# HoangChuongNguyen/ibgs

Hardware: AMD Instinct MI355X
Metric: train-step fps (fwd+bwd raster) @1080p, 1M Gaussians (higher is better)
Workload: dtype f32

## Files before the change

ibgs_amd/csrc/api.hip:

```cpp
#include "common.h"
#include "sh_color.h"
#include <sched.h>
#include <time.h>
#include <string.h>
#include <cstdlib>
#include <stdlib.h>
#include <stdio.h>
#include <cstdarg>
#include <cstdio>
#include <cstring>
#include <vector>
#include <map>
#include <mutex>

namespace ibgs {

static thread_local char g_err[512] = "";
void set_error(const char* fmt, ...)
{
    va_list ap; va_start(ap, fmt);
    vsnprintf(g_err, sizeof(g_err), fmt, ap);
    va_end(ap);
}

// ... 464 lines not shown
    if (a.render_geo) {
        if (a.plane_mode == IBGS_PLANE_NONE ? (!a.all_map || !a.dL_dall_map)
                                            : (a.plane_mode == IBGS_PLANE_LEARNT ? (!a.plane_normal || !a.dL_dplane_normal)
                                                                                 : (a.plane_mode != IBGS_PLANE_SMALLEST_AXIS || !a.scales || !a.rotations))) {
            set_error("geo backward: plane inputs / gradient outputs missing"); return -IBGS_ERR_INVALID;
        }
        if (!a.out_depth || !a.out_warped || !a.ref_to_src || !a.src_images) { set_error("geo backward inputs missing"); return -IBGS_ERR_INVALID; }
        if (!a.tex || a.tex_bytes < ibgs_required_tex(a.n_src, a.W, a.H)) { set_error("tex scratch too small"); return -IBGS_ERR_ALLOC; }
        if (!a.geo_table || a.geo_table_bytes < (a.buffer_length > 0 ? ibgs_required_geo_table_for(a.W, a.H, a.buffer_length) : ibgs_required_geo_table(a.W, a.H))) { set_error("geo_table scratch too small"); return -IBGS_ERR_ALLOC; }
    }
    int rc;
    GeomState g = GeomState::carve(a.geom, (size_t)a.P, nullptr);
    ImgState im = ImgState::carve(a.img, a.W, a.H, nullptr);
    BinState b = BinState::carve(a.binning, (size_t)a.R, a.W, a.H, nullptr);
    const float4* rgba = nullptr;
    float* geo_tab = nullptr;
    if (a.render_geo) {
        float4* t = reinterpret_cast<float4*>((reinterpret_cast<uintptr_t>(a.tex) + 127) & ~uintptr_t(127));
        const bool window = a.dL_ddepth || a.dL_dwarped;
        if (window && !(a.flags & IBGS_FLAG_TEX_PACKED) && (rc = launch_pack_rgba(s, a.src_images, t, a.W, a.H, a.n_src))) return rc;
        rgba = t;
        geo_tab = reinterpret_cast<float*>((reinterpret_cast<uintptr_t>(a.geo_table) + 127) & ~uintptr_t(127));
    }
    if (a.R > 0) {
        const bool det = (a.flags & IBGS_FLAG_DETERMINISTIC) != 0;
        DetState ds{};
        int ipt = 1;
        if (det) {
            if (!a.det_scratch || a.det_scratch_bytes < ibgs_required_deterministic_for(a.R, a.P, a.W, a.H, a.render_geo, a.flags)) { set_error("det_scratch too small"); return -IBGS_ERR_ALLOC; }
            ipt = render_backward_waves_per_tile(a);
            ds = DetState::carve(a.det_scratch, (size_t)a.R * ipt, (size_t)a.P, nullptr);
            if ((rc = launch_det_prepare(s, ds, (size_t)a.R * ipt))) return rc;
        }
        if ((rc = launch_render_backward(s, a, g, b, im, rgba, det ? ds.slab : nullptr, geo_tab))) return rc;
        if (det) { StageTimer t(s, IBGS_STAGE_TILE_ORDER); if ((rc = launch_det_reduce(s, ds, b.point_list, (size_t)a.R, ipt, a.P, a.grad_acc, g.offsets + a.P))) return rc; }
        if ((rc = stage_check(s, debug, "render backward"))) return rc;
    }
    { StageTimer t(s, IBGS_STAGE_PREPROCESS_BWD); if ((rc = launch_preprocess_backward(s, a, g))) return rc; }
    if ((rc = stage_check(s, debug, "preprocess backward"))) return rc;
    return check_sort_flag(rs, true);
}

int32_t ibgs_sh_grad_from_views(void* stream, int32_t P, int32_t D, int32_t M, int32_t n_views, const float* means3D,
                                const float* camposes, const float* dcolor, int64_t view_stride, float* dL_dsh)
{
    if (view_stride == 0) view_stride = (int64_t)P * 3;
    if (view_stride < (int64_t)P * 3) { set_error("view_stride smaller than P x 3"); return -IBGS_ERR_INVALID; }
    if (P <= 0 || M <= 0) return 0;
    if (D < 0 || D > 3 || (D + 1) * (D + 1) > M || n_views < 0) { set_error("bad SH degree / view count"); return -IBGS_ERR_INVALID; }
    if (!means3D || !dL_dsh || (n_views > 0 && (!camposes || !dcolor))) { set_error("null pointer"); return -IBGS_ERR_INVALID; }
    return launch_sh_grad_from_views(reinterpret_cast<hipStream_t>(stream), P, D, M, n_views, means3D, camposes, dcolor, (size_t)view_stride, dL_dsh);
}

int32_t ibgs_mark_visible(void* stream, int32_t P, const float* means3D, const float* viewmatrix,
                          const float* projmatrix, uint8_t* present)
{
    (void)projmatrix;
    if (P <= 0) return 0;
    if (!means3D || !viewmatrix || !present) { set_error("null pointer"); return -IBGS_ERR_INVALID; }
    return launch_mark_visible(reinterpret_cast<hipStream_t>(stream), P, means3D, viewmatrix, present);
}
// ... 3 lines not shown
```

ibgs_amd/csrc/common.h:

```cpp
#pragma once
#include <hip/hip_runtime.h>
#include <stdint.h>
#include <stddef.h>
#include <stdlib.h>
#include "../../include/ibgs_rast.h"

namespace ibgs {

constexpr int TILE = IBGS_TILE;
constexpr int WAVE = 64;
constexpr int REC_FLOATS = 16;
constexpr int GACC_FLOATS = 16;
constexpr bool grad_acc_offsets_fit32(long long P) { return P >= 0 && P <= (1ll << 32) / (long long)(GACC_FLOATS * sizeof(float)); }

constexpr int IBGS_CULL_WORDS = 4;
constexpr int IBGS_CULL_MAX_TILES = 64 * IBGS_CULL_WORDS;

enum RecField { R_X = 0, R_Y = 1, R_OP = 2, R_PAD0 = 3, R_CA = 4, R_CB = 5, R_CC = 6, R_DIST = 7,
                R_R = 8, R_G = 9, R_B = 10, R_PAD1 = 11, R_NX = 12, R_NY = 13, R_NZ = 14, R_PAD2 = 15 };

enum GaccField { G_SX = 0, G_SY = 1, G_AX = 2, G_AY = 3, G_SXX = 4, G_SXY = 5, G_SYY = 6, G_S0 = 7,
                 G_R = 8, G_G = 9, G_B = 10, G_NX = 11, G_NY = 12, G_NZ = 13, G_DIST = 14, G_PAD = 15 };

struct Carver {
// ... 330 lines not shown
                     uint32_t* result_alt = nullptr, const ShRide* ride = nullptr);
bool radix_takes_sh_ride(size_t n, int nbits);
void radix_set_sh_ride(bool on);
size_t radix_zero_elems(size_t n, int nbits);
int exclusive_scan_u32(hipStream_t s, const uint32_t* in, uint32_t* out, size_t n, uint32_t* scratch,
                       size_t scratch_elems, bool with_total);
size_t scan_scratch_elems(size_t n);
int radix_set_onesweep(int mode);
void radix_set_lookback_spins(uint32_t v);

int launch_binning(hipStream_t s, int P, int64_t cap, int gx, int gy, const GeomState& g, const BinState& b, uint32_t* ranges,
                   const uint32_t* order_hint = nullptr, uint32_t* meta = nullptr ,
                   int n_views = 1 ,
                   const uint32_t* sort_flag = nullptr, uint32_t* host_note = nullptr ,
                   uint32_t note_ticket = 0 );
constexpr int ORDER_CLASSES = 1024;
int launch_binning_scatter(hipStream_t s, int64_t cap, int gx, int gy, const BinState& b);

int launch_pack_rgba(hipStream_t s, const float* src, float4* dst, int W, int H, int n);
constexpr int GEO_TAB_FIELDS = 6;
inline size_t geo_table_floats(int W, int H) { return (size_t)W * H * IBGS_MAX_BUFFER_LENGTH * GEO_TAB_FIELDS; }
int launch_render_forward(hipStream_t s, const ibgs_forward_args& a, const GeomState& g, const BinState& b,
                          const ImgState& im, const float4* src_rgba);
int launch_render_backward(hipStream_t s, const ibgs_backward_args& a, const GeomState& g, const BinState& b,
                           const ImgState& im, const float4* src_rgba, float* slab = nullptr, float* geo_tab = nullptr);
int launch_preprocess_backward(hipStream_t s, const ibgs_backward_args& a, const GeomState& g);

struct DetState {
    float* slab;
    uint32_t* keys[2];
    uint32_t* vals[2];
    uint32_t* seg;
    uint32_t* hist; size_t hist_elems;
    static DetState carve(char* base, size_t rows, size_t P, size_t* total);
};
int render_backward_waves_per_tile(const ibgs_backward_args& a);
int render_backward_ref_arith(uint32_t flags);
int launch_det_prepare(hipStream_t s, const DetState& d, size_t rows);
int launch_det_reduce(hipStream_t s, const DetState& d, const uint32_t* point_list, size_t R, int ipt, int P, float* gacc, const uint32_t* listed );
int launch_sh_grad_from_views(hipStream_t s, int P, int D, int M, int n_views, const float* means3D, const float* camposes,
                              const float* dcolor, size_t view_stride, float* dL_dsh);

__device__ __forceinline__ uint32_t pack_rect(int lo, int hi) { return (uint32_t)lo | ((uint32_t)hi << 16); }

}
```

ibgs_amd/csrc/preprocess_bwd.hip:

```cpp
#include "common.h"
#include "adam_math.h"

namespace ibgs {

__constant__ float bC1 = 0.4886025119029199f;
__constant__ float bC0 = 0.28209479177387814f;
__constant__ float bC2[5] = {1.0925484305920792f, -1.0925484305920792f, 0.31539156525252005f,
                             -1.0925484305920792f, 0.5462742152960396f};
__constant__ float bC3[7] = {-0.5900435899266435f, 2.890611442640554f, -0.4570457994644658f,
                             0.3731763325901154f, -0.4570457994644658f, 1.445305721320277f,
                             -0.5900435899266435f};

struct PreBwdParams {
    int P, D, M;
    const float* means3D; const int32_t* radii; const float* shs; const float* shs_rest; const uint8_t* clamped;
    const float* scales; const float* rotations; float scale_modifier;
    const float* cov3D;
    float* gacc;
    int clear_gacc;
    int risky_rows;
    const float* rec;
    float* dL_dmean2D; float* dL_dmean2D_abs; float* dL_dconic; float* dL_dopacity; float* dL_dcolors;
    float* dL_dall_map; float* dL_dmean3D; float* dL_dcov3D; float* dL_dsh; float* dL_dsh_rest; float* dL_dscale; float* dL_drot;
    const float* plane_normal; const float* plane_offset; int plane_mode;
    float* dL_dplane_normal; float* dL_dplane_offset;
};

__device__ __forceinline__ int sh_basis(int D, float x, float y, float z, float (&B)[16])
{
    int nb = 1;
    B[0] = bC0;
    const float xx = x * x, yy = y * y, zz = z * z, xy = x * y, yz = y * z, xz = x * z;
    if (D > 0) {
        B[1] = -bC1 * y; B[2] = bC1 * z; B[3] = -bC1 * x; nb = 4;
        if (D > 1) {
            B[4] = bC2[0] * xy; B[5] = bC2[1] * yz; B[6] = bC2[2] * (2.0f * zz - xx - yy);
            B[7] = bC2[3] * xz; B[8] = bC2[4] * (xx - yy); nb = 9;
            if (D > 2) {
                B[9] = bC3[0] * y * (3.0f * xx - yy); B[10] = bC3[1] * xy * z;
                B[11] = bC3[2] * y * (4.0f * zz - xx - yy);
                B[12] = bC3[3] * z * (2.0f * zz - 3.0f * xx - 3.0f * yy);
                B[13] = bC3[4] * x * (4.0f * zz - xx - yy); B[14] = bC3[5] * z * (xx - yy);
                B[15] = bC3[6] * x * (xx - 3.0f * yy); nb = 16;
            }
        }
    }
    return nb;
}

template <bool FAST16, bool WRITE_SH, bool SPLIT = false>
__global__ void __launch_bounds__(FAST16 ? 64 : 256) preprocess_bwd_kernel(PreBwdParams p, Cam cam)
{
    __shared__ float4 s_t[FAST16 ? 64 * 13 : 1];
    const int i = blockIdx.x * blockDim.x + threadIdx.x;
    const bool valid = i < p.P;
    bool vis = valid && (p.radii[i] > 0);
    float4 g0 = make_float4(0.f, 0.f, 0.f, 0.f), g1 = g0, g2 = g0, g3 = g0;
    if (vis) {
        float4* grow = reinterpret_cast<float4*>(p.gacc + (size_t)i * GACC_FLOATS);
        g0 = grow[0]; g1 = grow[1]; g2 = grow[2]; g3 = grow[3];
        const uint32_t any = (__float_as_uint(g0.x) | __float_as_uint(g0.y) | __float_as_uint(g0.z) | __float_as_uint(g0.w) |
                              __float_as_uint(g1.x) | __float_as_uint(g1.y) | __float_as_uint(g1.z) | __float_as_uint(g1.w) |
                              __float_as_uint(g2.x) | __float_as_uint(g2.y) | __float_as_uint(g2.z) | __float_as_uint(g2.w) |
                              __float_as_uint(g3.x) | __float_as_uint(g3.y) | __float_as_uint(g3.z) | __float_as_uint(g3.w)) & 0x7FFFFFFFu;
        if (any == 0u) vis = false;
        else if (p.clear_gacc) { const float4 z = make_float4(0.f, 0.f, 0.f, 0.f); grow[0] = z; grow[1] = z; grow[2] = z; grow[3] = z; }
    }
    float gv[(FAST16 && WRITE_SH) ? 48 : 1];
    if (FAST16 && WRITE_SH) {
#pragma unroll
        for (int k = 0; k < 48; k++) gv[k] = 0.f;
    }
    if (valid && !vis) {
        p.dL_dmean2D[3 * i] = 0.f; p.dL_dmean2D[3 * i + 1] = 0.f; p.dL_dmean2D[3 * i + 2] = 0.f;
        if (p.dL_dmean2D_abs) { p.dL_dmean2D_abs[3 * i] = 0.f; p.dL_dmean2D_abs[3 * i + 1] = 0.f; p.dL_dmean2D_abs[3 * i + 2] = 0.f; }
        if (p.dL_dconic) { p.dL_dconic[4 * i] = 0.f; p.dL_dconic[4 * i + 1] = 0.f; p.dL_dconic[4 * i + 2] = 0.f; p.dL_dconic[4 * i + 3] = 0.f; }
        p.dL_dopacity[i] = 0.f;
        if (p.dL_dcolors) { p.dL_dcolors[3 * i] = 0.f; p.dL_dcolors[3 * i + 1] = 0.f; p.dL_dcolors[3 * i + 2] = 0.f; }
        if (p.dL_dall_map) for (int k = 0; k < 5; k++) p.dL_dall_map[5 * i + k] = 0.f;
        if (p.dL_dplane_normal) { p.dL_dplane_normal[3 * i] = 0.f; p.dL_dplane_normal[3 * i + 1] = 0.f; p.dL_dplane_normal[3 * i + 2] = 0.f; }
        if (p.dL_dplane_offset) p.dL_dplane_offset[i] = 0.f;
        p.dL_dmean3D[3 * i] = 0.f; p.dL_dmean3D[3 * i + 1] = 0.f; p.dL_dmean3D[3 * i + 2] = 0.f;
        if (p.dL_dcov3D) for (int k = 0; k < 6; k++) p.dL_dcov3D[6 * i + k] = 0.f;
        if (!FAST16 && WRITE_SH && p.shs) {
            if (SPLIT) {
                float* gd = p.dL_dsh + (size_t)i * 3; float* gr = p.dL_dsh_rest + (size_t)i * (p.M - 1) * 3;
                gd[0] = gd[1] = gd[2] = 0.f;
                for (int k = 0; k < 3 * (p.M - 1); k++) gr[k] = 0.f;
            } else { float* gsh = p.dL_dsh + (size_t)i * p.M * 3; for (int k = 0; k < 3 * p.M; k++) gsh[k] = 0.f; }
        }
        if (p.scales) {
            p.dL_dscale[3 * i] = 0.f; p.dL_dscale[3 * i + 1] = 0.f; p.dL_dscale[3 * i + 2] = 0.f;
            p.dL_drot[4 * i] = 0.f; p.dL_drot[4 * i + 1] = 0.f; p.dL_drot[4 * i + 2] = 0.f; p.dL_drot[4 * i + 3] = 0.f;
        }
    }
    if (FAST16 && SPLIT && p.shs) {
// ... 280 lines not shown
#pragma unroll
        for (int r = 0; r < 3; r++) p.dL_dscale[3 * i + r] = R[0][r] * dM[r][0] + R[1][r] * dM[r][1] + R[2][r] * dM[r][2];
#pragma unroll
        for (int r = 0; r < 3; r++)
#pragma unroll
            for (int cc = 0; cc < 3; cc++) G[r][cc] = sv[r] * dM[r][cc];
        p.dL_drot[4 * i + 0] = prot[0] + 2 * z * (G[0][1] - G[1][0]) + 2 * y * (G[2][0] - G[0][2]) + 2 * x * (G[1][2] - G[2][1]);
        p.dL_drot[4 * i + 1] = prot[1] + 2 * y * (G[1][0] + G[0][1]) + 2 * z * (G[2][0] + G[0][2]) + 2 * r_ * (G[1][2] - G[2][1]) - 4 * x * (G[2][2] + G[1][1]);
        p.dL_drot[4 * i + 2] = prot[2] + 2 * x * (G[1][0] + G[0][1]) + 2 * r_ * (G[2][0] - G[0][2]) + 2 * z * (G[1][2] + G[2][1]) - 4 * y * (G[2][2] + G[0][0]);
        p.dL_drot[4 * i + 3] = prot[3] + 2 * r_ * (G[0][1] - G[1][0]) + 2 * x * (G[2][0] + G[0][2]) + 2 * y * (G[1][2] + G[2][1]) - 4 * z * (G[1][1] + G[0][0]);
    }
    }

    if (FAST16 && WRITE_SH && SPLIT && p.shs) {
        const int lane = threadIdx.x;
        __syncthreads();
        float* s_w = reinterpret_cast<float*>(s_t);
        s_w[2880 + 3 * lane] = gv[0]; s_w[2880 + 3 * lane + 1] = gv[1]; s_w[2880 + 3 * lane + 2] = gv[2];
#pragma unroll
        for (int k = 0; k < 45; k++) s_w[45 * lane + k] = gv[3 + k];
        __syncthreads();
        const int i0 = blockIdx.x * 64;
        const int nrows = min(64, p.P - i0);
        float4* dr = reinterpret_cast<float4*>(p.dL_dsh_rest + (size_t)i0 * 45);
        float4* dd = reinterpret_cast<float4*>(p.dL_dsh + (size_t)i0 * 3);
#pragma unroll
        for (int it = 0; it < 12; it++) {
            const int q = it * 64 + lane;
            const float4 f4 = s_t[q];
            const float f[4] = {f4.x, f4.y, f4.z, f4.w};
            if (q < 720) {
                if (4 * q + 3 < nrows * 45) dr[q] = f4;
                else { float* op = p.dL_dsh_rest + (size_t)i0 * 45; for (int k = 0; k < 4; k++) if (4 * q + k < nrows * 45) op[4 * q + k] = f[k]; }
            } else {
                const int qd = q - 720;
                if (4 * qd + 3 < nrows * 3) dd[qd] = f4;
                else { float* op = p.dL_dsh + (size_t)i0 * 3; for (int k = 0; k < 4; k++) if (4 * qd + k < nrows * 3) op[4 * qd + k] = f[k]; }
            }
        }
    } else if (FAST16 && WRITE_SH && p.shs) {
        const int lane = threadIdx.x;
#pragma unroll
        for (int v = 0; v < 12; v++) s_t[lane * 13 + v] = make_float4(gv[4 * v], gv[4 * v + 1], gv[4 * v + 2], gv[4 * v + 3]);
        __syncthreads();
        const int i0 = blockIdx.x * 64;
        const int nrows = min(64, p.P - i0);
        float4* dst = reinterpret_cast<float4*>(p.dL_dsh + (size_t)i0 * 48);
#pragma unroll
        for (int k = 0; k < 12; k++) {
            const int f = lane + 64 * k;
            const int r = f / 12, c = f - 12 * r;
            if (r < nrows) dst[f] = s_t[r * 13 + c];
        }
    }
}

int launch_preprocess_backward(hipStream_t s, const ibgs_backward_args& a, const GeomState& g)
{
    PreBwdParams p;
    p.P = a.P; p.D = a.D; p.M = a.M;
    p.means3D = a.means3D; p.radii = a.radii; p.shs = a.shs; p.shs_rest = a.shs_rest; p.clamped = g.clamped;
    p.scales = a.scales; p.rotations = a.rotations; p.scale_modifier = a.scale_modifier;
    p.cov3D = a.cov3D_precomp ? a.cov3D_precomp : g.cov3D;
    p.gacc = a.grad_acc; p.rec = g.rec; p.clear_gacc = (a.flags & IBGS_FLAG_CLEAR_GRAD_ACC) ? 1 : 0;
    { const int ra = render_backward_ref_arith(a.flags); p.risky_rows = (ra & 4) ? 2 : ((ra & 2) ? 1 : 0); }
    p.dL_dmean2D = a.dL_dmean2D; p.dL_dmean2D_abs = a.dL_dmean2D_abs; p.dL_dconic = a.dL_dconic;
    p.dL_dopacity = a.dL_dopacity; p.dL_dcolors = a.dL_dcolors; p.dL_dall_map = a.dL_dall_map;
    p.dL_dmean3D = a.dL_dmean3D; p.dL_dcov3D = a.dL_dcov3D; p.dL_dsh = a.dL_dsh; p.dL_dsh_rest = a.dL_dsh_rest; p.dL_dscale = a.dL_dscale; p.dL_drot = a.dL_drot;
    p.plane_normal = a.plane_normal; p.plane_offset = a.plane_offset; p.plane_mode = a.plane_mode;
    p.dL_dplane_normal = a.dL_dplane_normal; p.dL_dplane_offset = a.dL_dplane_offset;
    const Cam cam = make_cam(a.viewmatrix, a.projmatrix, a.campos, a.bg, a.tanfovx, a.tanfovy, a.W, a.H);
    const bool factored = a.shs && (a.flags & IBGS_FLAG_SH_FACTORED);
    const bool split = a.shs && a.shs_rest;
    if (a.shs && a.M == 16) {
        if (factored && split) hipLaunchKernelGGL((preprocess_bwd_kernel<true, false, true>), dim3((a.P + 63) / 64), dim3(64), 0, s, p, cam);
        else if (factored) hipLaunchKernelGGL((preprocess_bwd_kernel<true, false>), dim3((a.P + 63) / 64), dim3(64), 0, s, p, cam);
        else if (split) hipLaunchKernelGGL((preprocess_bwd_kernel<true, true, true>), dim3((a.P + 63) / 64), dim3(64), 0, s, p, cam);
        else hipLaunchKernelGGL((preprocess_bwd_kernel<true, true>), dim3((a.P + 63) / 64), dim3(64), 0, s, p, cam);
    } else {
        if (factored && split) hipLaunchKernelGGL((preprocess_bwd_kernel<false, false, true>), dim3((a.P + 255) / 256), dim3(256), 0, s, p, cam);
        else if (factored) hipLaunchKernelGGL((preprocess_bwd_kernel<false, false>), dim3((a.P + 255) / 256), dim3(256), 0, s, p, cam);
        else if (split) hipLaunchKernelGGL((preprocess_bwd_kernel<false, true, true>), dim3((a.P + 255) / 256), dim3(256), 0, s, p, cam);
        else hipLaunchKernelGGL((preprocess_bwd_kernel<false, true>), dim3((a.P + 255) / 256), dim3(256), 0, s, p, cam);
    }
    IBGS_HIP(hipGetLastError());
    return 0;
}

template <bool FAST16>
__global__ void __launch_bounds__(FAST16 ? 64 : 256) sh_grad_from_views_kernel(int P, int D, int M, int n_views, size_t view_stride, const float* __restrict__ means3D,
                                                                                const float* __restrict__ camposes, const float* __restrict__ dcolor,
                                                                                float* __restrict__ dL_dsh)
{
// ... 144 lines not shown
```

ibgs_amd/csrc/render_bwd.hip:

```cpp
#include "common.h"
#include <stdlib.h>
#include "wave_reduce.h"
#include <type_traits>

namespace ibgs {

struct BwdParams {
    const uint32_t* ranges; const uint32_t* point_list; const float4* rec;
    Cam cam;
    int ntiles;
    TileMap tmap;
    int n_src; int tex_quant;
    int power_skip;
    const uint32_t* tile_risky;
    const float* ref_to_src; const float4* src_rgba;
    const float* final_T; const uint32_t* n_contrib; const float* sum_w; const uint32_t* low_high;
    const int32_t* valid_idx; const float* valid_w;
    const float* depth_pixels; const float* warped_pixels;
    const float* dL_dcolor; const float* dL_dnormal; const float* dL_ddepth; const float* dL_dwarped;
    float* gacc;
    int tab_slots;
    const uint32_t* slot_c; const uint32_t* meta; float* tab;
    const uint32_t* order;
    int slab_ipt;
    int hybrid_grid1;
    int acc32;
    float* slab;
};

__device__ __forceinline__ float quant8b(float a, int quant) { return quant ? floorf(a * 256.0f + 0.5f) * (1.0f / 256.0f) : a; }

__device__ __forceinline__ float4 tex_rgba_b(const float4* __restrict__ img, int W, int H, float x, float y, int quant)
{
#pragma clang fp contract(off)
    const float xb = x - 0.5f, yb = y - 0.5f;
    const float fxi = floorf(xb), fyi = floorf(yb);
    const float a = quant8b(xb - fxi, quant), b = quant8b(yb - fyi, quant);
    const int i0 = min(W - 1, max(0, (int)fxi)), i1 = min(W - 1, max(0, (int)fxi + 1));
    const int j0 = min(H - 1, max(0, (int)fyi)), j1 = min(H - 1, max(0, (int)fyi + 1));
    const float4 t00 = img[(size_t)j0 * W + i0], t10 = img[(size_t)j0 * W + i1];
    const float4 t01 = img[(size_t)j1 * W + i0], t11 = img[(size_t)j1 * W + i1];
    const float w00 = (1.f - a) * (1.f - b), w10 = a * (1.f - b), w01 = (1.f - a) * b, w11 = a * b;
    float4 r;
    r.x = w00 * t00.x + w10 * t10.x + w01 * t01.x + w11 * t11.x;
    r.y = w00 * t00.y + w10 * t10.y + w01 * t01.y + w11 * t11.y;
    r.z = w00 * t00.z + w10 * t10.z + w01 * t01.z + w11 * t11.z;
    r.w = 1.0f;
    return r;
}

__device__ __forceinline__ uint32_t wave_max_u32(uint32_t v)
// ... 637 lines not shown
                    v[2] = aX; v[3] = aY;
                    v[8] = vR; v[9] = vG; v[10] = vB; v[11] = vNx; v[12] = vNy; v[13] = vNz; v[14] = vD; v[15] = 0.f;
                    const float tot = wave_transpose_reduce16(v, lane);
                    const uint32_t id = __float_as_uint(q0.w);
                    if (col >= 0) {
                        if (p.slab) p.slab[((size_t)(r0 + k) * (p.slab_ipt ? p.slab_ipt : IPT) + (size_t)sub) * GACC_FLOATS + col] = tot;
                        else atomicAdd(p.gacc + (size_t)id * GACC_FLOATS + col, tot);
                    }
                }
            }
        };
        if (bg0) { if (stable) chunk(std::true_type{}, std::true_type{}); else chunk(std::false_type{}, std::true_type{}); }
        else { if (stable) chunk(std::true_type{}, std::false_type{}); else chunk(std::false_type{}, std::false_type{}); }
        __syncthreads();
        top -= count;
    }
}

#ifdef IBGS_TRACE_WAVES
__device__ uint4 g_trace_bwd[IBGS_TRACE_MAX];
#endif
__global__ void __launch_bounds__(64, 8) render_bwd_color_kernel(BwdParams p)
{
    IBGS_TRACE_BEGIN();
    int tile, sub = 0;
    bool have;
    if (p.order) { const uint32_t t = p.order[blockIdx.x]; tile = (int)(t & ~ORDER_SPLIT_BIT); have = t != 0xFFFFFFFFu; }
    else have = tile_map_item(p.tmap, blockIdx.x, p.cam.gx, p.cam.gy, 1, tile, sub);
    __shared__ float4 s_rec[3][BWD_CHUNK];
    __shared__ __align__(16) unsigned char s_pix[4 * WAVE * sizeof(float4)];
    if (have && !tile_is_risky(p.tile_risky, tile)) render_bwd_color_body<4, true, false, true>(p, tile, sub, s_rec, reinterpret_cast<float4 (*)[WAVE]>(s_pix));
    IBGS_TRACE_END(g_trace_bwd);
}
__global__ void __launch_bounds__(64, 8) render_bwd_color_noabs_kernel(BwdParams p)
{
    int tile, sub = 0;
    bool have;
    if (p.order) { const uint32_t t = p.order[blockIdx.x]; tile = (int)(t & ~ORDER_SPLIT_BIT); have = t != 0xFFFFFFFFu; }
    else have = tile_map_item(p.tmap, blockIdx.x, p.cam.gx, p.cam.gy, 1, tile, sub);
    __shared__ float4 s_rec[3][BWD_CHUNK];
    __shared__ __align__(16) unsigned char s_pix[4 * WAVE * sizeof(float4)];
    if (have && !tile_is_risky(p.tile_risky, tile)) render_bwd_color_body<4, false, false, true>(p, tile, sub, s_rec, reinterpret_cast<float4 (*)[WAVE]>(s_pix));
}
template <bool ABS>
__global__ void __launch_bounds__(64, 4) render_bwd_color_risk_kernel(BwdParams p)
{
    __shared__ float4 s_rec[3][BWD_CHUNK];
    __shared__ float4 s_gpix[4][WAVE];
    int tile = (int)blockIdx.x;
    if (p.order) { const uint32_t t = p.order[blockIdx.x]; if (t == 0xFFFFFFFFu) return; tile = (int)(t & ~ORDER_SPLIT_BIT); }
    if (tile >= p.ntiles || !tile_is_risky(p.tile_risky, tile)) return;
    render_bwd_color_body<4, ABS, true>(p, tile, 0, s_rec, s_gpix);
}

constexpr int ORDER_SNAKE_ROUNDS = 8;
__global__ void __launch_bounds__(1024) tile_order_kernel(int ntiles, int nslots , int slot_rounds ,
                                                          const uint32_t* __restrict__ walked_waves, const uint32_t* __restrict__ meta, uint32_t* __restrict__ order,
                                                          uint32_t* __restrict__ order_out ,
// ... 44 lines not shown
    uint32_t before = 0;
    for (int ww = 0; ww < wave; ww++) before += s_w[ww];
    s_hist[tid] = before + inc - v;
    __syncthreads();
    const uint32_t nrounds = (uint32_t)nslots / (uint32_t)ORDER_CLASSES;
    auto put = [&](int t, uint32_t key) {
        const uint32_t r = atomicAdd(&s_hist[bucket(key)], 1u);
        const uint32_t stratum = r / ORDER_CLASSES, c = r % ORDER_CLASSES;
        uint32_t slot = r;
        if (nrounds <= (uint32_t)slot_rounds) {
            const uint32_t round = (stratum + 1u) % nrounds;
            slot = round * ORDER_CLASSES + ((stratum & 1u) ? ORDER_CLASSES - 1u - c : c);
        }
        const uint32_t word = (uint32_t)t | ((theta_pct > 0 && hybrid_split(key, total, (uint32_t)theta_pct)) ? ORDER_SPLIT_BIT : 0u);
        order[slot] = word;
        if (order_out) order_out[slot] = word;
    };
#pragma unroll
    for (int k = 0; k < KEEP; k++) if (tid + k * 1024 < ntiles) put(tid + k * 1024, w[k]);
    for (int t = tid + KEEP * 1024; t < ntiles; t += 1024) put(t, walked_of(t));
}
__global__ void __launch_bounds__(64, 8) render_bwd_color_small_kernel(BwdParams p)
{
    int tile, sub;
    __shared__ float4 s_rec[3][BWD_CHUNK];
    __shared__ float4 s_gpix[1][WAVE];
    if (tile_map_item(p.tmap, blockIdx.x, p.cam.gx, p.cam.gy, 4, tile, sub) && !tile_is_risky(p.tile_risky, tile)) render_bwd_color_body<1>(p, tile, sub, s_rec, s_gpix);
}
template <bool ABS>
__global__ void __launch_bounds__(64, 8) render_bwd_color_hybrid_kernel(BwdParams p)
{
    __shared__ float4 s_rec[3][BWD_CHUNK];
    __shared__ float4 s_gpix[4][WAVE];
    int tile, sub; bool split;
    if (!hybrid_item(blockIdx.x, p.hybrid_grid1, p.order, tile, sub, split) || tile_is_risky(p.tile_risky, tile)) return;
    if (split) render_bwd_color_body<1, ABS>(p, tile, sub, s_rec, s_gpix);
    else if (sub == 0) render_bwd_color_body<4, ABS>(p, tile, 0, s_rec, s_gpix);
}
template <int PPL, bool ABS>
__device__ __forceinline__ void render_bwd_geo_entry(const BwdParams& p)
{
    __shared__ float4 s_rec[4][BWD_CHUNK];
    __shared__ float4 s_gpix[PPL][WAVE];
    __shared__ float4 s_gnrm[PPL][WAVE];
    int tile, sub;
    if (PPL == 4 && p.order) { const uint32_t t = p.order[blockIdx.x]; if (t == 0xFFFFFFFFu) return; tile = (int)(t & ~ORDER_SPLIT_BIT); sub = 0; }
    else if (!tile_map_item(p.tmap, blockIdx.x, p.cam.gx, p.cam.gy, 4 / PPL, tile, sub)) return;
    if (tile_is_risky(p.tile_risky, tile)) return;
    render_bwd_geo_body<PPL, ABS>(p, tile, sub, s_rec, s_gpix, s_gnrm);
}
template <bool ABS>
__global__ void __launch_bounds__(64, 3) render_bwd_geo_risk_kernel(BwdParams p)
{
    __shared__ float4 s_rec[4][BWD_CHUNK];
    __shared__ float4 s_gpix[4][WAVE];
    __shared__ float4 s_gnrm[4][WAVE];
    int tile = (int)blockIdx.x;
    if (p.order) { const uint32_t t = p.order[blockIdx.x]; if (t == 0xFFFFFFFFu) return; tile = (int)(t & ~ORDER_SPLIT_BIT); }
    if (tile >= p.ntiles || !tile_is_risky(p.tile_risky, tile)) return;
    render_bwd_geo_body<4, ABS, true>(p, tile, 0, s_rec, s_gpix, s_gnrm);
}
__global__ void __launch_bounds__(64, 4) render_bwd_geo4_kernel(BwdParams p) { render_bwd_geo_entry<4, true>(p); }
__global__ void __launch_bounds__(64, 4) render_bwd_geo4_noabs_kernel(BwdParams p) { render_bwd_geo_entry<4, false>(p); }
__global__ void __launch_bounds__(64, 6) render_bwd_geo_kernel(BwdParams p) { render_bwd_geo_entry<1, true>(p); }
template <bool ABS>
__global__ void __launch_bounds__(64, 4) render_bwd_geo_hybrid_kernel(BwdParams p)
{
    __shared__ float4 s_rec[4][BWD_CHUNK];
    __shared__ float4 s_gpix[4][WAVE];
    __shared__ float4 s_gnrm[4][WAVE];
    int tile, sub; bool split;
    if (!hybrid_item(blockIdx.x, p.hybrid_grid1, p.order, tile, sub, split) || tile_is_risky(p.tile_risky, tile)) return;
    if (split) render_bwd_geo_body<1, ABS>(p, tile, sub, s_rec, s_gpix, s_gnrm);
    else if (sub == 0) render_bwd_geo_body<4, ABS>(p, tile, 0, s_rec, s_gpix, s_gnrm);
}

int render_backward_ref_arith(uint32_t flags)
{
    if (flags & IBGS_FLAG_NO_REF_POWER_SKIP) return 0;
    return RA_DECIDE | ((flags & IBGS_FLAG_REF_ARITH) ? RA_ASSOC : RA_LFORM);
}

int render_backward_waves_per_tile(const ibgs_backward_args& a)
{
    const int nt = ((a.W + TILE - 1) / TILE) * ((a.H + TILE - 1) / TILE);
    if (a.render_geo) return ((a.flags & IBGS_FLAG_QUADRANT_WAVES) ? false : ((a.flags & IBGS_FLAG_TILE_WAVES) ? true : nt >= 4096)) ? 1 : 4;
    return ((a.flags & IBGS_FLAG_QUADRANT_WAVES) ? true : ((a.flags & IBGS_FLAG_TILE_WAVES) ? false : nt < hybrid_max_tiles())) ? 4 : 1;
}

int launch_render_backward(hipStream_t s, const ibgs_backward_args& a, const GeomState& g, const BinState& b,
                           const ImgState& im, const float4* src_rgba, float* slab, float* geo_tab)
{
    BwdParams p;
    p.ranges = im.ranges; p.point_list = b.point_list; p.rec = reinterpret_cast<const float4*>(g.rec);
    p.cam = make_cam(a.viewmatrix, a.projmatrix, a.campos, a.bg, a.tanfovx, a.tanfovy, a.W, a.H);
    p.ntiles = p.cam.gx * p.cam.gy;
    p.n_src = a.n_src; p.tex_quant = (a.flags & IBGS_FLAG_TEX_QUANT) ? 1 : 0;
    p.power_skip = render_backward_ref_arith(a.flags);
    p.tile_risky = (p.power_skip & RA_ASSOC) ? im.tile_risky : nullptr;
    p.ref_to_src = a.ref_to_src; p.src_rgba = src_rgba;
    p.final_T = im.final_T; p.n_contrib = im.n_contrib; p.sum_w = im.sum_w; p.low_high = im.low_high;
    p.valid_idx = im.valid_idx; p.valid_w = im.valid_w;
    p.depth_pixels = a.out_depth; p.warped_pixels = a.out_warped;
    p.dL_dcolor = a.dL_dcolor; p.dL_dnormal = a.dL_dnormal; p.dL_ddepth = a.dL_ddepth; p.dL_dwarped = a.dL_dwarped;
    p.gacc = a.grad_acc; p.acc32 = grad_acc_offsets_fit32((long long)a.P) ? 1 : 0; p.slab = slab; p.order = nullptr; p.slab_ipt = 0; p.hybrid_grid1 = 0;
    p.slot_c = im.slot_c; p.meta = im.meta; p.tab = geo_tab;
    p.tab_slots = (a.buffer_length >= 1 && a.buffer_length < IBGS_MAX_BUFFER_LENGTH) ? a.buffer_length + 1 : IBGS_MAX_BUFFER_LENGTH;
    const int nt = p.ntiles;
    p.tmap = a.render_geo ? TileMap{TMAP_BLOCK, 1, 8, 4} : TileMap{TMAP_BLOCK, 1, 8, 8};
    auto grid = [&](int ipt) { return dim3((unsigned)tile_map_grid(p.tmap, p.cam.gx, p.cam.gy, ipt)); };
    auto launch_risk = [&](int nslots_or_0) {
        if (!p.tile_risky) return;
        BwdParams r = p;
        r.slab_ipt = render_backward_waves_per_tile(a);
        r.hybrid_grid1 = 0;
        if (nslots_or_0 == 0) r.order = nullptr;
        const dim3 g((unsigned)(nslots_or_0 ? nslots_or_0 : nt));
        StageTimer t(s, IBGS_STAGE_RENDER_BWD);
        const bool noabs = (a.flags & IBGS_FLAG_NO_ABS_GRAD) != 0;
        if (a.render_geo) { if (noabs) hipLaunchKernelGGL(render_bwd_geo_risk_kernel<false>, g, dim3(64), 0, s, r); else hipLaunchKernelGGL(render_bwd_geo_risk_kernel<true>, g, dim3(64), 0, s, r); }
        else { if (noabs) hipLaunchKernelGGL(render_bwd_color_risk_kernel<false>, g, dim3(64), 0, s, r); else hipLaunchKernelGGL(render_bwd_color_risk_kernel<true>, g, dim3(64), 0, s, r); }
    };
    const bool noabs = (a.flags & IBGS_FLAG_NO_ABS_GRAD) != 0;
    const int nslots = (nt + ORDER_CLASSES - 1) / ORDER_CLASSES * ORDER_CLASSES;
    auto launch_order = [&](int slot_rounds, int theta) {
        StageTimer t(s, IBGS_STAGE_TILE_ORDER);
        hipLaunchKernelGGL(tile_order_kernel, dim3(1), dim3(1024), 0, s, nt, nslots, slot_rounds, im.tile_walked, im.meta, im.tile_order, a.tile_order_out, theta);
        p.order = im.tile_order;
    };
    int risk_slots = 0;
    if (a.render_geo) {
        const bool big = (a.flags & IBGS_FLAG_QUADRANT_WAVES) ? false : ((a.flags & IBGS_FLAG_TILE_WAVES) ? true : nt >= 4096);
        const bool window = a.dL_ddepth || a.dL_dwarped;
        if (window && !geo_tab) { set_error("geo backward needs the window table scratch"); return -IBGS_ERR_INVALID; }
        if (window) {
            StageTimer t(s, IBGS_STAGE_GEO_WINDOW);
            hipLaunchKernelGGL(geo_window_kernel, dim3((unsigned)(((size_t)a.W * a.H + 255) / 256)), dim3(256), 0, s, p);
        } else p.tab = nullptr;
        IBGS_HIP(hipGetLastError());
        if (big) {
            launch_order(4, 0);
            risk_slots = nslots;
            StageTimer t(s, IBGS_STAGE_RENDER_BWD);
            if (noabs) hipLaunchKernelGGL(render_bwd_geo4_noabs_kernel, dim3((unsigned)nslots), dim3(64), 0, s, p);
            else hipLaunchKernelGGL(render_bwd_geo4_kernel, dim3((unsigned)nslots), dim3(64), 0, s, p);
        } else if (!(a.flags & IBGS_FLAG_QUADRANT_WAVES) && nt >= HYBRID_MIN_TILES) {
            launch_order(4, hybrid_theta());
            IBGS_HIP(hipGetLastError());
            p.slab_ipt = 4; p.hybrid_grid1 = nslots;
            risk_slots = nslots;
            StageTimer t(s, IBGS_STAGE_RENDER_BWD);
            if (noabs) hipLaunchKernelGGL(render_bwd_geo_hybrid_kernel<false>, dim3(4u * (unsigned)nslots), dim3(64), 0, s, p);
            else hipLaunchKernelGGL(render_bwd_geo_hybrid_kernel<true>, dim3(4u * (unsigned)nslots), dim3(64), 0, s, p);
        } else {
            StageTimer t(s, IBGS_STAGE_RENDER_BWD);
            hipLaunchKernelGGL(render_bwd_geo_kernel, grid(4), dim3(64), 0, s, p);
        }
    } else if ((a.flags & IBGS_FLAG_QUADRANT_WAVES) ? true : ((a.flags & IBGS_FLAG_TILE_WAVES) ? false : nt < hybrid_max_tiles())) {
        if (!(a.flags & IBGS_FLAG_QUADRANT_WAVES) && nt >= HYBRID_MIN_TILES) {
            launch_order(ORDER_SNAKE_ROUNDS, hybrid_theta());
            IBGS_HIP(hipGetLastError());
            p.slab_ipt = 4; p.hybrid_grid1 = nslots;
            risk_slots = nslots;
            StageTimer t(s, IBGS_STAGE_RENDER_BWD);
            if (noabs) hipLaunchKernelGGL(render_bwd_color_hybrid_kernel<false>, dim3(4u * (unsigned)nslots), dim3(64), 0, s, p);
            else hipLaunchKernelGGL(render_bwd_color_hybrid_kernel<true>, dim3(4u * (unsigned)nslots), dim3(64), 0, s, p);
        } else {
            StageTimer t(s, IBGS_STAGE_RENDER_BWD);
            hipLaunchKernelGGL(render_bwd_color_small_kernel, grid(4), dim3(64), 0, s, p);
        }
    } else {
        launch_order(ORDER_SNAKE_ROUNDS, 0);
        IBGS_HIP(hipGetLastError());
        risk_slots = nslots;
        StageTimer t(s, IBGS_STAGE_RENDER_BWD);
        if (noabs) hipLaunchKernelGGL(render_bwd_color_noabs_kernel, dim3((unsigned)nslots), dim3(64), 0, s, p);
        else hipLaunchKernelGGL(render_bwd_color_kernel, dim3((unsigned)nslots), dim3(64), 0, s, p);
    }
    IBGS_HIP(hipGetLastError());
    launch_risk(risk_slots);
    IBGS_HIP(hipGetLastError());
    return 0;
}

}

#ifdef IBGS_COUNT_LANES
extern "C" int ibgs_debug_lanes_bwd(unsigned long long* dst, int reset)
{
    int rc = (int)hipMemcpyFromSymbol(dst, HIP_SYMBOL(ibgs::g_lanes_bwd), sizeof(unsigned long long) * 4, 0, hipMemcpyDeviceToHost);
    if (reset) { unsigned long long z[4] = {0, 0, 0, 0}; rc |= (int)hipMemcpyToSymbol(HIP_SYMBOL(ibgs::g_lanes_bwd), z, sizeof(z), 0, hipMemcpyHostToDevice); }
    return rc;
}
#endif
#ifdef IBGS_TRACE_WAVES
extern "C" int ibgs_debug_trace_bwd(void* dst, size_t bytes)
{
    return (int)hipMemcpyFromSymbol(dst, HIP_SYMBOL(ibgs::g_trace_bwd), bytes < sizeof(uint4) * ibgs::IBGS_TRACE_MAX ? bytes : sizeof(uint4) * ibgs::IBGS_TRACE_MAX, 0, hipMemcpyDeviceToHost);
}
#endif
// ... 1 lines not shown
```

Measured before the change: 636.0.

## Zero offscreen Gaussian gradients as passenger blocks inside render backward

Appends extra workgroups to the render-backward grid that zero the gradient rows of Gaussians with non-positive radii. Preprocess-backward then skips those writes, including the SH row stores. The aim is to hide the zeroing stores of culled points under the raster backward tail instead of paying for them in preprocess backward. This adds blocks to the backward launch and couples the two kernels' write responsibilities. The SH transpose store masking also adds per-store predicate arithmetic.

```diff
diff --git a/ibgs_amd/csrc/api.hip b/ibgs_amd/csrc/api.hip
--- a/ibgs_amd/csrc/api.hip
+++ b/ibgs_amd/csrc/api.hip
@@ -1,5 +1,6 @@
 #include "common.h"
 #include "sh_color.h"
+#include "zero_rows.h"
 #include <sched.h>
 #include <time.h>
 #include <string.h>
@@ -510,6 +511,7 @@
         rgba = t;
         geo_tab = reinterpret_cast<float*>((reinterpret_cast<uintptr_t>(a.geo_table) + 127) & ~uintptr_t(127));
     }
+    bool offscreen_done = false;
     if (a.R > 0) {
         const bool det = (a.flags & IBGS_FLAG_DETERMINISTIC) != 0;
         DetState ds{};
@@ -520,11 +522,13 @@
             ds = DetState::carve(a.det_scratch, (size_t)a.R * ipt, (size_t)a.P, nullptr);
             if ((rc = launch_det_prepare(s, ds, (size_t)a.R * ipt))) return rc;
         }
-        if ((rc = launch_render_backward(s, a, g, b, im, rgba, det ? ds.slab : nullptr, geo_tab))) return rc;
+        const ZeroRows zr = zero_rows_of(a);
+        if ((rc = launch_render_backward(s, a, g, b, im, rgba, det ? ds.slab : nullptr, geo_tab, &zr))) return rc;
+        offscreen_done = true;
         if (det) { StageTimer t(s, IBGS_STAGE_TILE_ORDER); if ((rc = launch_det_reduce(s, ds, b.point_list, (size_t)a.R, ipt, a.P, a.grad_acc, g.offsets + a.P))) return rc; }
         if ((rc = stage_check(s, debug, "render backward"))) return rc;
     }
-    { StageTimer t(s, IBGS_STAGE_PREPROCESS_BWD); if ((rc = launch_preprocess_backward(s, a, g))) return rc; }
+    { StageTimer t(s, IBGS_STAGE_PREPROCESS_BWD); if ((rc = launch_preprocess_backward(s, a, g, offscreen_done))) return rc; }
     if ((rc = stage_check(s, debug, "preprocess backward"))) return rc;
     return check_sort_flag(rs, true);
 }
diff --git a/ibgs_amd/csrc/common.h b/ibgs_amd/csrc/common.h
--- a/ibgs_amd/csrc/common.h
+++ b/ibgs_amd/csrc/common.h
@@ -376,9 +376,10 @@
 inline size_t geo_table_floats(int W, int H) { return (size_t)W * H * IBGS_MAX_BUFFER_LENGTH * GEO_TAB_FIELDS; }
 int launch_render_forward(hipStream_t s, const ibgs_forward_args& a, const GeomState& g, const BinState& b,
                           const ImgState& im, const float4* src_rgba);
+struct ZeroRows;
 int launch_render_backward(hipStream_t s, const ibgs_backward_args& a, const GeomState& g, const BinState& b,
-                           const ImgState& im, const float4* src_rgba, float* slab = nullptr, float* geo_tab = nullptr);
-int launch_preprocess_backward(hipStream_t s, const ibgs_backward_args& a, const GeomState& g);
+                           const ImgState& im, const float4* src_rgba, float* slab = nullptr, float* geo_tab = nullptr, const ZeroRows* zero_rows = nullptr);
+int launch_preprocess_backward(hipStream_t s, const ibgs_backward_args& a, const GeomState& g, bool offscreen_done = false);
 
 struct DetState {
     float* slab;
diff --git a/ibgs_amd/csrc/preprocess_bwd.hip b/ibgs_amd/csrc/preprocess_bwd.hip
--- a/ibgs_amd/csrc/preprocess_bwd.hip
+++ b/ibgs_amd/csrc/preprocess_bwd.hip
@@ -24,6 +24,7 @@
     float* dL_dall_map; float* dL_dmean3D; float* dL_dcov3D; float* dL_dsh; float* dL_dsh_rest; float* dL_dscale; float* dL_drot;
     const float* plane_normal; const float* plane_offset; int plane_mode;
     float* dL_dplane_normal; float* dL_dplane_offset;
+    int offscreen_done;
 };
 
 __device__ __forceinline__ int sh_basis(int D, float x, float y, float z, float (&B)[16])
@@ -55,6 +56,7 @@
     const int i = blockIdx.x * blockDim.x + threadIdx.x;
     const bool valid = i < p.P;
     bool vis = valid && (p.radii[i] > 0);
+    const bool done = valid && !vis && p.offscreen_done;
     float4 g0 = make_float4(0.f, 0.f, 0.f, 0.f), g1 = g0, g2 = g0, g3 = g0;
     if (vis) {
         float4* grow = reinterpret_cast<float4*>(p.gacc + (size_t)i * GACC_FLOATS);
@@ -71,7 +73,7 @@
 #pragma unroll
         for (int k = 0; k < 48; k++) gv[k] = 0.f;
     }
-    if (valid && !vis) {
+    if (valid && !vis && !done) {
         p.dL_dmean2D[3 * i] = 0.f; p.dL_dmean2D[3 * i + 1] = 0.f; p.dL_dmean2D[3 * i + 2] = 0.f;
         if (p.dL_dmean2D_abs) { p.dL_dmean2D_abs[3 * i] = 0.f; p.dL_dmean2D_abs[3 * i + 1] = 0.f; p.dL_dmean2D_abs[3 * i + 2] = 0.f; }
         if (p.dL_dconic) { p.dL_dconic[4 * i] = 0.f; p.dL_dconic[4 * i + 1] = 0.f; p.dL_dconic[4 * i + 2] = 0.f; p.dL_dconic[4 * i + 3] = 0.f; }
@@ -398,6 +400,7 @@
         __syncthreads();
         const int i0 = blockIdx.x * 64;
         const int nrows = min(64, p.P - i0);
+        const uint64_t todo = ~__builtin_amdgcn_ballot_w64(done);
         float4* dr = reinterpret_cast<float4*>(p.dL_dsh_rest + (size_t)i0 * 45);
         float4* dd = reinterpret_cast<float4*>(p.dL_dsh + (size_t)i0 * 3);
 #pragma unroll
@@ -406,10 +409,13 @@
             const float4 f4 = s_t[q];
             const float f[4] = {f4.x, f4.y, f4.z, f4.w};
             if (q < 720) {
+                const int ra = (4 * q) / 45, rb = min((4 * q + 3) / 45, 63);
+                if (!(((todo >> ra) | (todo >> rb)) & 1ull)) continue;
                 if (4 * q + 3 < nrows * 45) dr[q] = f4;
                 else { float* op = p.dL_dsh_rest + (size_t)i0 * 45; for (int k = 0; k < 4; k++) if (4 * q + k < nrows * 45) op[4 * q + k] = f[k]; }
             } else {
-                const int qd = q - 720;
+                const int qd = q - 720, ra = (4 * qd) / 3, rb = (4 * qd + 3) / 3;
+                if (!(((todo >> ra) | (todo >> rb)) & 1ull)) continue;
                 if (4 * qd + 3 < nrows * 3) dd[qd] = f4;
                 else { float* op = p.dL_dsh + (size_t)i0 * 3; for (int k = 0; k < 4; k++) if (4 * qd + k < nrows * 3) op[4 * qd + k] = f[k]; }
             }
@@ -421,17 +427,18 @@
         __syncthreads();
         const int i0 = blockIdx.x * 64;
         const int nrows = min(64, p.P - i0);
+        const uint64_t todo = ~__builtin_amdgcn_ballot_w64(done);
         float4* dst = reinterpret_cast<float4*>(p.dL_dsh + (size_t)i0 * 48);
 #pragma unroll
         for (int k = 0; k < 12; k++) {
             const int f = lane + 64 * k;
             const int r = f / 12, c = f - 12 * r;
-            if (r < nrows) dst[f] = s_t[r * 13 + c];
-        }
-    }
-}
-
-int launch_preprocess_backward(hipStream_t s, const ibgs_backward_args& a, const GeomState& g)
+            if (r < nrows && ((todo >> r) & 1ull)) dst[f] = s_t[r * 13 + c];
+        }
+    }
+}
+
+int launch_preprocess_backward(hipStream_t s, const ibgs_backward_args& a, const GeomState& g, bool offscreen_done)
 {
     PreBwdParams p;
     p.P = a.P; p.D = a.D; p.M = a.M;
@@ -445,6 +452,7 @@
     p.dL_dmean3D = a.dL_dmean3D; p.dL_dcov3D = a.dL_dcov3D; p.dL_dsh = a.dL_dsh; p.dL_dsh_rest = a.dL_dsh_rest; p.dL_dscale = a.dL_dscale; p.dL_drot = a.dL_drot;
     p.plane_normal = a.plane_normal; p.plane_offset = a.plane_offset; p.plane_mode = a.plane_mode;
     p.dL_dplane_normal = a.dL_dplane_normal; p.dL_dplane_offset = a.dL_dplane_offset;
+    p.offscreen_done = offscreen_done ? 1 : 0;
     const Cam cam = make_cam(a.viewmatrix, a.projmatrix, a.campos, a.bg, a.tanfovx, a.tanfovy, a.W, a.H);
     const bool factored = a.shs && (a.flags & IBGS_FLAG_SH_FACTORED);
     const bool split = a.shs && a.shs_rest;
diff --git a/ibgs_amd/csrc/render_bwd.hip b/ibgs_amd/csrc/render_bwd.hip
--- a/ibgs_amd/csrc/render_bwd.hip
+++ b/ibgs_amd/csrc/render_bwd.hip
@@ -1,6 +1,7 @@
 #include "common.h"
 #include <stdlib.h>
 #include "wave_reduce.h"
+#include "zero_rows.h"
 #include <type_traits>
 
 namespace ibgs {
@@ -26,7 +27,14 @@
     int hybrid_grid1;
     int acc32;
     float* slab;
+    ZeroRows zr;
 };
+__device__ __forceinline__ bool bwd_passenger(const BwdParams& p)
+{
+    if ((int)blockIdx.x < p.zr.wg0) return false;
+    zero_rows_passenger(p.zr, (int)blockIdx.x - p.zr.wg0);
+    return true;
+}
 
 __device__ __forceinline__ float quant8b(float a, int quant) { return quant ? floorf(a * 256.0f + 0.5f) * (1.0f / 256.0f) : a; }
 
@@ -710,6 +718,7 @@
 #endif
 __global__ void __launch_bounds__(64, 8) render_bwd_color_kernel(BwdParams p)
 {
+    if (bwd_passenger(p)) return;
     IBGS_TRACE_BEGIN();
     int tile, sub = 0;
     bool have;
@@ -722,6 +731,7 @@
 }
 __global__ void __launch_bounds__(64, 8) render_bwd_color_noabs_kernel(BwdParams p)
 {
+    if (bwd_passenger(p)) return;
     int tile, sub = 0;
     bool have;
     if (p.order) { const uint32_t t = p.order[blockIdx.x]; tile = (int)(t & ~ORDER_SPLIT_BIT); have = t != 0xFFFFFFFFu; }
@@ -812,6 +822,7 @@
 }
 __global__ void __launch_bounds__(64, 8) render_bwd_color_small_kernel(BwdParams p)
 {
+    if (bwd_passenger(p)) return;
     int tile, sub;
     __shared__ float4 s_rec[3][BWD_CHUNK];
     __shared__ float4 s_gpix[1][WAVE];
@@ -822,6 +833,7 @@
 {
     __shared__ float4 s_rec[3][BWD_CHUNK];
     __shared__ float4 s_gpix[4][WAVE];
+    if (bwd_passenger(p)) return;
     int tile, sub; bool split;
     if (!hybrid_item(blockIdx.x, p.hybrid_grid1, p.order, tile, sub, split) || tile_is_risky(p.tile_risky, tile)) return;
     if (split) render_bwd_color_body<1, ABS>(p, tile, sub, s_rec, s_gpix);
@@ -833,6 +845,7 @@
     __shared__ float4 s_rec[4][BWD_CHUNK];
     __shared__ float4 s_gpix[PPL][WAVE];
     __shared__ float4 s_gnrm[PPL][WAVE];
+    if (bwd_passenger(p)) return;
     int tile, sub;
     if (PPL == 4 && p.order) { const uint32_t t = p.order[blockIdx.x]; if (t == 0xFFFFFFFFu) return; tile = (int)(t & ~ORDER_SPLIT_BIT); sub = 0; }
     else if (!tile_map_item(p.tmap, blockIdx.x, p.cam.gx, p.cam.gy, 4 / PPL, tile, sub)) return;
@@ -859,6 +872,7 @@
     __shared__ float4 s_rec[4][BWD_CHUNK];
     __shared__ float4 s_gpix[4][WAVE];
     __shared__ float4 s_gnrm[4][WAVE];
+    if (bwd_passenger(p)) return;
     int tile, sub; bool split;
     if (!hybrid_item(blockIdx.x, p.hybrid_grid1, p.order, tile, sub, split) || tile_is_risky(p.tile_risky, tile)) return;
     if (split) render_bwd_geo_body<1, ABS>(p, tile, sub, s_rec, s_gpix, s_gnrm);
@@ -879,7 +893,7 @@
 }
 
 int launch_render_backward(hipStream_t s, const ibgs_backward_args& a, const GeomState& g, const BinState& b,
-                           const ImgState& im, const float4* src_rgba, float* slab, float* geo_tab)
+                           const ImgState& im, const float4* src_rgba, float* slab, float* geo_tab, const ZeroRows* zero_rows)
 {
     BwdParams p;
     p.ranges = im.ranges; p.point_list = b.point_list; p.rec = reinterpret_cast<const float4*>(g.rec);
@@ -896,12 +910,17 @@
     p.gacc = a.grad_acc; p.acc32 = grad_acc_offsets_fit32((long long)a.P) ? 1 : 0; p.slab = slab; p.order = nullptr; p.slab_ipt = 0; p.hybrid_grid1 = 0;
     p.slot_c = im.slot_c; p.meta = im.meta; p.tab = geo_tab;
     p.tab_slots = (a.buffer_length >= 1 && a.buffer_length < IBGS_MAX_BUFFER_LENGTH) ? a.buffer_length + 1 : IBGS_MAX_BUFFER_LENGTH;
+    const int n_zero = zero_rows ? zero_rows_blocks(zero_rows->P) : 0;
+    if (zero_rows) p.zr = *zero_rows; else p.zr = ZeroRows{};
+    p.zr.wg0 = ZR_NONE;
+    auto with = [&](dim3 tiles) { p.zr.wg0 = n_zero ? (int)tiles.x : ZR_NONE; return dim3(tiles.x + (unsigned)n_zero); };
     const int nt = p.ntiles;
     p.tmap = a.render_geo ? TileMap{TMAP_BLOCK, 1, 8, 4} : TileMap{TMAP_BLOCK, 1, 8, 8};
     auto grid = [&](int ipt) { return dim3((unsigned)tile_map_grid(p.tmap, p.cam.gx, p.cam.gy, ipt)); };
     auto launch_risk = [&](int nslots_or_0) {
         if (!p.tile_risky) return;
         BwdParams r = p;
+        r.zr.wg0 = ZR_NONE;
         r.slab_ipt = render_backward_waves_per_tile(a);
         r.hybrid_grid1 = 0;
         if (nslots_or_0 == 0) r.order = nullptr;
@@ -932,19 +951,22 @@
             launch_order(4, 0);
             risk_slots = nslots;
             StageTimer t(s, IBGS_STAGE_RENDER_BWD);
-            if (noabs) hipLaunchKernelGGL(render_bwd_geo4_noabs_kernel, dim3((unsigned)nslots), dim3(64), 0, s, p);
-            else hipLaunchKernelGGL(render_bwd_geo4_kernel, dim3((unsigned)nslots), dim3(64), 0, s, p);
+            const dim3 gr = with(dim3((unsigned)nslots));
+            if (noabs) hipLaunchKernelGGL(render_bwd_geo4_noabs_kernel, gr, dim3(64), 0, s, p);
+            else hipLaunchKernelGGL(render_bwd_geo4_kernel, gr, dim3(64), 0, s, p);
         } else if (!(a.flags & IBGS_FLAG_QUADRANT_WAVES) && nt >= HYBRID_MIN_TILES) {
             launch_order(4, hybrid_theta());
             IBGS_HIP(hipGetLastError());
             p.slab_ipt = 4; p.hybrid_grid1 = nslots;
             risk_slots = nslots;
             StageTimer t(s, IBGS_STAGE_RENDER_BWD);
-            if (noabs) hipLaunchKernelGGL(render_bwd_geo_hybrid_kernel<false>, dim3(4u * (unsigned)nslots), dim3(64), 0, s, p);
-            else hipLaunchKernelGGL(render_bwd_geo_hybrid_kernel<true>, dim3(4u * (unsigned)nslots), dim3(64), 0, s, p);
+            const dim3 gr = with(dim3(4u * (unsigned)nslots));
+            if (noabs) hipLaunchKernelGGL(render_bwd_geo_hybrid_kernel<false>, gr, dim3(64), 0, s, p);
+            else hipLaunchKernelGGL(render_bwd_geo_hybrid_kernel<true>, gr, dim3(64), 0, s, p);
         } else {
             StageTimer t(s, IBGS_STAGE_RENDER_BWD);
-            hipLaunchKernelGGL(render_bwd_geo_kernel, grid(4), dim3(64), 0, s, p);
+            const dim3 gr = with(grid(4));
+            hipLaunchKernelGGL(render_bwd_geo_kernel, gr, dim3(64), 0, s, p);
         }
     } else if ((a.flags & IBGS_FLAG_QUADRANT_WAVES) ? true : ((a.flags & IBGS_FLAG_TILE_WAVES) ? false : nt < hybrid_max_tiles())) {
         if (!(a.flags & IBGS_FLAG_QUADRANT_WAVES) && nt >= HYBRID_MIN_TILES) {
@@ -953,19 +975,22 @@
             p.slab_ipt = 4; p.hybrid_grid1 = nslots;
             risk_slots = nslots;
             StageTimer t(s, IBGS_STAGE_RENDER_BWD);
-            if (noabs) hipLaunchKernelGGL(render_bwd_color_hybrid_kernel<false>, dim3(4u * (unsigned)nslots), dim3(64), 0, s, p);
-            else hipLaunchKernelGGL(render_bwd_color_hybrid_kernel<true>, dim3(4u * (unsigned)nslots), dim3(64), 0, s, p);
+            const dim3 gr = with(dim3(4u * (unsigned)nslots));
+            if (noabs) hipLaunchKernelGGL(render_bwd_color_hybrid_kernel<false>, gr, dim3(64), 0, s, p);
+            else hipLaunchKernelGGL(render_bwd_color_hybrid_kernel<true>, gr, dim3(64), 0, s, p);
         } else {
             StageTimer t(s, IBGS_STAGE_RENDER_BWD);
-            hipLaunchKernelGGL(render_bwd_color_small_kernel, grid(4), dim3(64), 0, s, p);
+            const dim3 gr = with(grid(4));
+            hipLaunchKernelGGL(render_bwd_color_small_kernel, gr, dim3(64), 0, s, p);
         }
     } else {
         launch_order(ORDER_SNAKE_ROUNDS, 0);
         IBGS_HIP(hipGetLastError());
         risk_slots = nslots;
         StageTimer t(s, IBGS_STAGE_RENDER_BWD);
-        if (noabs) hipLaunchKernelGGL(render_bwd_color_noabs_kernel, dim3((unsigned)nslots), dim3(64), 0, s, p);
-        else hipLaunchKernelGGL(render_bwd_color_kernel, dim3((unsigned)nslots), dim3(64), 0, s, p);
+        const dim3 gr = with(dim3((unsigned)nslots));
+        if (noabs) hipLaunchKernelGGL(render_bwd_color_noabs_kernel, gr, dim3(64), 0, s, p);
+        else hipLaunchKernelGGL(render_bwd_color_kernel, gr, dim3(64), 0, s, p);
     }
     IBGS_HIP(hipGetLastError());
     launch_risk(risk_slots);
diff --git a/ibgs_amd/csrc/zero_rows.h b/ibgs_amd/csrc/zero_rows.h
--- /dev/null
+++ b/ibgs_amd/csrc/zero_rows.h
@@ -0,0 +1,103 @@
+#pragma once
+#include "common.h"
+
+namespace ibgs {
+
+constexpr int ZR_BLOCK = 1024;
+constexpr int ZR_NONE = 0x7FFFFFFF;
+
+struct ZeroRows {
+    int wg0;
+    int P;
+    const int32_t* radii;
+    float* mean2D; float* mean2D_abs; float* conic; float* opacity; float* colors; float* all_map;
+    float* plane_normal; float* plane_offset; float* mean3D; float* cov3D; float* scale; float* rot;
+    float* sh; float* sh_rest;
+    int sh_words, rest_words;
+};
+
+inline int zero_rows_blocks(int P) { return (P + ZR_BLOCK - 1) / ZR_BLOCK; }
+
+inline ZeroRows zero_rows_of(const ibgs_backward_args& a)
+{
+    ZeroRows z{};
+    z.wg0 = ZR_NONE; z.P = a.P; z.radii = a.radii;
+    z.mean2D = a.dL_dmean2D; z.mean2D_abs = a.dL_dmean2D_abs; z.conic = a.dL_dconic; z.opacity = a.dL_dopacity; z.colors = a.dL_dcolors;
+    z.all_map = a.dL_dall_map; z.plane_normal = a.dL_dplane_normal; z.plane_offset = a.dL_dplane_offset;
+    z.mean3D = a.dL_dmean3D; z.cov3D = a.dL_dcov3D;
+    if (a.scales) { z.scale = a.dL_dscale; z.rot = a.dL_drot; }
+    if (a.shs && !(a.flags & IBGS_FLAG_SH_FACTORED)) {
+        if (a.shs_rest) { z.sh = a.dL_dsh; z.sh_words = 3; z.sh_rest = a.dL_dsh_rest; z.rest_words = 3 * (a.M - 1); }
+        else { z.sh = a.dL_dsh; z.sh_words = 3 * a.M; }
+    }
+    return z;
+}
+
+#ifdef __HIPCC__
+template <int RW>
+__device__ __forceinline__ void zero_wide_rows(float* __restrict__ base, int rw_rt, int i0, int nrows, uint64_t off, int lane)
+{
+    const int rw = RW ? RW : rw_rt;
+    float* blk = base + (size_t)i0 * rw;
+    const int total = nrows * rw;
+    const bool aligned = (reinterpret_cast<uintptr_t>(blk) & 15u) == 0;
+    for (int w0 = 4 * lane; w0 < total; w0 += 4 * 64) {
+        int r = w0 / rw, rem = w0 - r * rw;
+        bool o[4];
+#pragma unroll
+        for (int k = 0; k < 4; k++) {
+            o[k] = (w0 + k < total) && ((off >> r) & 1ull);
+            if (++rem == rw) { rem = 0; r++; }
+        }
+        if (aligned && o[0] && o[1] && o[2] && o[3]) *reinterpret_cast<float4*>(blk + w0) = make_float4(0.f, 0.f, 0.f, 0.f);
+        else {
+#pragma unroll
+            for (int k = 0; k < 4; k++) if (o[k]) blk[w0 + k] = 0.f;
+        }
+    }
+}
+__device__ __forceinline__ void zero_wide(float* __restrict__ base, int rw, int i0, int nrows, uint64_t off, int lane)
+{
+    if (rw == 48) zero_wide_rows<48>(base, rw, i0, nrows, off, lane);
+    else if (rw == 45) zero_wide_rows<45>(base, rw, i0, nrows, off, lane);
+    else if (rw == 3) zero_wide_rows<3>(base, rw, i0, nrows, off, lane);
+    else zero_wide_rows<0>(base, rw, i0, nrows, off, lane);
+}
+
+__device__ __forceinline__ void zero_rows_passenger(const ZeroRows& z, int block)
+{
+    const int lane = (int)threadIdx.x;
+    const int first = block * ZR_BLOCK;
+    if (first >= z.P) return;
+    const int count = min(ZR_BLOCK, z.P - first);
+    int32_t rad = lane < count ? z.radii[first + lane] : 1;
+    for (int k0 = 0; k0 < count; k0 += 64) {
+        const int i0 = first + k0, i = i0 + lane;
+        const bool mine = k0 + lane < count && rad <= 0;
+        if (k0 + 64 + lane < count) rad = z.radii[i + 64];
+        const uint64_t off = __builtin_amdgcn_ballot_w64(mine);
+        if (off == 0ull) continue;
+        if (mine) {
+            z.mean2D[3 * (size_t)i] = 0.f; z.mean2D[3 * (size_t)i + 1] = 0.f; z.mean2D[3 * (size_t)i + 2] = 0.f;
+            if (z.mean2D_abs) { z.mean2D_abs[3 * (size_t)i] = 0.f; z.mean2D_abs[3 * (size_t)i + 1] = 0.f; z.mean2D_abs[3 * (size_t)i + 2] = 0.f; }
+            if (z.conic) { z.conic[4 * (size_t)i] = 0.f; z.conic[4 * (size_t)i + 1] = 0.f; z.conic[4 * (size_t)i + 2] = 0.f; z.conic[4 * (size_t)i + 3] = 0.f; }
+            z.opacity[i] = 0.f;
+            if (z.colors) { z.colors[3 * (size_t)i] = 0.f; z.colors[3 * (size_t)i + 1] = 0.f; z.colors[3 * (size_t)i + 2] = 0.f; }
+            if (z.all_map) for (int k = 0; k < 5; k++) z.all_map[5 * (size_t)i + k] = 0.f;
+            if (z.plane_normal) { z.plane_normal[3 * (size_t)i] = 0.f; z.plane_normal[3 * (size_t)i + 1] = 0.f; z.plane_normal[3 * (size_t)i + 2] = 0.f; }
+            if (z.plane_offset) z.plane_offset[i] = 0.f;
+            z.mean3D[3 * (size_t)i] = 0.f; z.mean3D[3 * (size_t)i + 1] = 0.f; z.mean3D[3 * (size_t)i + 2] = 0.f;
+            if (z.cov3D) for (int k = 0; k < 6; k++) z.cov3D[6 * (size_t)i + k] = 0.f;
+            if (z.scale) {
+                z.scale[3 * (size_t)i] = 0.f; z.scale[3 * (size_t)i + 1] = 0.f; z.scale[3 * (size_t)i + 2] = 0.f;
+                z.rot[4 * (size_t)i] = 0.f; z.rot[4 * (size_t)i + 1] = 0.f; z.rot[4 * (size_t)i + 2] = 0.f; z.rot[4 * (size_t)i + 3] = 0.f;
+            }
+        }
+        const int nrows = min(64, count - k0);
+        if (z.sh) zero_wide(z.sh, z.sh_words, i0, nrows, off, lane);
+        if (z.sh_rest) zero_wide(z.sh_rest, z.rest_words, i0, nrows, off, lane);
+    }
+}
+#endif
+
+}
```

Result: no change. 634.9 (-0.2%).
